# AER-RC/monoRTM

Measured on AMD Instinct MI355X. Metric: (wavenumber x layer x line) optical-depth evals/sec, higher is better.
Workload: dtype f64; 1 GPU; c4: configs[3] whole: 1024 synthetic sonde profiles x 64 layers x 50 channels x 500 lines, f64, profile-sharded over 1 GPU(s): 1024 profiles on this rank; layers=64, wavenumbers=50, lines=500, nmol=7, launch=3 stream launches, parallelism=profile-sharded x1

## Files before the change

### monortm_amd/csrc/api.hip

```cpp
#include <algorithm>
#include <atomic>
#include <chrono>
#include <cmath>
#include <cstdlib>
#include <cstdio>
#include <cstring>
#include <dlfcn.h>
#include <functional>
#include <string>
#include <vector>

#include "device_common.hpp"
#include "line_table.hpp"
#include "modm_plan.hpp"
#include "lineshape.hpp"
#include "tables/monortm_tables.h"

namespace {
using namespace monortm_dev;

thread_local std::string g_init_error;

struct Ctx {
    int device = 0;
    int cus = 256;
    size_t phys_cap = 2ull << 30, far_cap = 1ull << 30;
    std::vector<Ctx *> shards;
    struct Opt : ModmPlanOpt {
        int ms_ablate = 0;
        double jac_dt = MONORTM_JAC_DT, jac_dlnw = MONORTM_JAC_DLNW;
    } opt;
    void *comm = nullptr;
    int comm_rank = 0, comm_world = 1;
    bool has_lines = false;
    int real_kind = 8;
    std::string err;
    monortm::LineTable host;
    DevLines lines{};
    DevTables tables{};
    std::vector<void *> owned;
    int *errflag = nullptr;
    void *partial = nullptr;
    monortm_dev::MwCache mw_cache;
    void *phys = nullptr;
    size_t phys_bytes = 0;
    void *far = nullptr;
    size_t far_bytes = 0;
    double lines_per_cm = 0.;
    bool no_physics_pass = false;
    hipStream_t far_stream = nullptr;
    hipEvent_t far_ev[2] = {nullptr, nullptr};
    double lc_frac = 0.;
    const int *ms_slot_base = nullptr;
    int ms_slot_host[MXMOL + 1] = {0};
    void *ms_scratch = nullptr;
    unsigned short *ms_reach = nullptr;
    size_t ms_scratch_bytes = 0;
    double *osum = nullptr;
    size_t osum_elems = 0;
    DevXsec xs{};
    std::vector<void *> xs_buf;
    struct Stage {
        void *p = nullptr;
        size_t bytes = 0;
    };
    Stage stage[12];
    void *jac_ws = nullptr;
    size_t jac_ws_bytes = 0;
    struct Obs {
        int handle = 0;
        int npath = 0, nwn = 0, nview = 0, nchan = 0;
        void *dev = nullptr;
        const int *view_start = nullptr, *mstart = nullptr, *mlane = nullptr;
        const double *wpath = nullptr, *mw = nullptr;
        std::vector<int> shard;
    };
    static constexpr int kMaxObs = 16;
    Obs obs[kMaxObs];
    hipStream_t hs = nullptr;
    int *errflag_host = nullptr;
    struct {
        const void *dev = nullptr, *host = nullptr;
// ... 25 lines not shown
    do {                                                                                             \
        hipError_t e_ = (call);                                                                      \
        if (e_ != hipSuccess) {                                                                      \
            (c)->err = std::string(#call) + ": " + hipGetErrorString(e_);                            \
            return MONORTM_EHIP;                                                                     \
        }                                                                                            \
    } while (0)

constexpr size_t kKernelCopyMax = 4u << 20;
__global__ __launch_bounds__(256) void copy16_kernel(const uint4 *__restrict__ src, uint4 *__restrict__ dst, size_t n16,
                                                     const uint4 *__restrict__ src2, uint4 *__restrict__ dst2, size_t n16b,
                                                     const int *flag_src, int *flag_dst) {
    for (size_t i = (size_t)blockIdx.x * 256 + threadIdx.x; i < n16; i += (size_t)gridDim.x * 256) dst[i] = src[i];
    if (blockIdx.x == gridDim.x - 1)
        for (size_t i = threadIdx.x; i < n16b; i += 256) dst2[i] = src2[i];
    if (flag_dst && blockIdx.x == 0 && threadIdx.x == 0) *flag_dst = *flag_src;
}
hipError_t move_arena(void *dst, const void *src, size_t bytes, hipMemcpyKind kind, hipStream_t s, const int *flag_src = nullptr,
                      int *flag_dst = nullptr, void *dst2 = nullptr, const void *src2 = nullptr, size_t bytes2 = 0) {
    if (bytes <= kKernelCopyMax) {
        const size_t n16 = bytes / 16;
        const unsigned blocks = (unsigned)std::min<size_t>(256, std::max<size_t>(1, (n16 + 255) / 256));
        hipLaunchKernelGGL(copy16_kernel, dim3(blocks), dim3(256), 0, s, static_cast<const uint4 *>(src), static_cast<uint4 *>(dst), n16,
                           static_cast<const uint4 *>(src2), static_cast<uint4 *>(dst2), bytes2 / 16, flag_src, flag_dst);
        return hipGetLastError();
    }
    hipError_t e = hipMemcpyAsync(dst, src, bytes, kind, s);
    if (e == hipSuccess && flag_dst) e = hipMemcpyAsync(flag_dst, flag_src, sizeof(int), hipMemcpyDeviceToHost, s);
    if (e == hipSuccess && bytes2) e = hipMemcpyAsync(dst2, src2, bytes2, hipMemcpyDefault, s);
    return e;
}

void comm_release(Ctx *c);

int set_option(Ctx *c, const char *name, const char *value) {
    const std::string n = name ? name : "", v = value ? value : "";
    const bool autov = v.empty() || v == "auto";
    long iv = 0;
    double dv = 0.;
    bool isint = false, isdbl = false;
    if (!autov) {
        char *end = nullptr;
        iv = strtol(v.c_str(), &end, 10);
        isint = end && end != v.c_str() && *end == '\0';
        end = nullptr;
        dv = strtod(v.c_str(), &end);
        isdbl = end && end != v.c_str() && *end == '\0';
    }
    if (n == "nslice" && (autov || (isint && iv >= 1 && iv <= 16))) c->opt.nslice = autov ? 0 : (int)iv;
    else if (n == "fair" && (autov || (isint && (iv == 0 || iv == 1)))) c->opt.fair = autov ? -1 : (int)iv;
    else if (n == "tile_waves" && (autov || (isint && (iv == 1 || iv == 2 || iv == 4)))) c->opt.tile_waves = autov ? 0 : (int)iv;
    else if (n == "far_levels" && (autov || (isint && iv >= 0 && iv <= FAR_MAXLEV))) c->opt.far_levels = autov ? -1 : (int)iv;
    else if (n == "lines_kernel" && (autov || v == "wn" || v == "ms")) c->opt.lines_ms = autov ? -1 : (v == "ms" ? 1 : 0);
#ifdef MONORTM_EXPERIMENT
    else if (n == "ms_ablate" && isint && iv >= 0 && iv <= 9) c->opt.ms_ablate = (int)iv;
#endif
    else if (n == "finish" && (autov || v == "generic")) c->opt.finish_generic = autov ? 0 : 1;
    else if (n == "ms_items" && (autov || (isint && (iv == 64 || iv == 128 || iv == 192 || iv == 256)))) c->opt.ms_items = autov ? 0 : (int)iv;
    else if ((n == "jac_dt" || n == "jac_dlnw") && (autov || (isdbl && std::isfinite(dv) && dv > 0. && (n == "jac_dt" || dv < 1.)))) {
        if (n == "jac_dt") c->opt.jac_dt = autov ? MONORTM_JAC_DT : dv;
        else c->opt.jac_dlnw = autov ? MONORTM_JAC_DLNW : dv;
    }
    else { c->err = "unknown option or value: " + n + " = " + v; return MONORTM_EARG; }
    return MONORTM_OK;
}

template <class T>
int upload(Ctx *c, const T *src, size_t n, const T **dst) {
    void *p = nullptr;
    const size_t bytes = std::max<size_t>(n, 1) * sizeof(T);
    HIPCHK(c, hipMalloc(&p, bytes));
    c->owned.push_back(p);
    if (n) HIPCHK(c, hipMemcpy(p, src, n * sizeof(T), hipMemcpyHostToDevice));
    *dst = static_cast<const T *>(p);
    return MONORTM_OK;
}

void prof_begin(Ctx *c, hipStream_t s, int k, Ctx::Ev &ev) {
    ev.k = -1;
    if (!((c->profiling >> k) & 1)) return;
    if (c->prof_stride > 1 && (c->prof_calls[k]++ % c->prof_stride) != 0) return;
    auto take = [&](hipEvent_t *e) {
        if (!c->event_pool.empty()) { *e = c->event_pool.back(); c->event_pool.pop_back(); }
        else hipEventCreate(e);
    };
    take(&ev.a);
    take(&ev.b);
    ev.k = k;
    hipEventRecord(ev.a, s);
}
void prof_end(Ctx *c, hipStream_t s, Ctx::Ev &ev) {
    if (ev.k < 0) return;
    hipEventRecord(ev.b, s);
    c->events.push_back(ev);
}

hipError_t grow(void **p, size_t *have, size_t need, size_t elem = 1) {
    if (need <= *have) return hipSuccess;
    hipError_t e = *p ? hipFree(*p) : hipSuccess;
    *p = nullptr;
    *have = 0;
    if (e == hipSuccess) e = hipMalloc(p, need * elem);
    if (e == hipSuccess) *have = need;
    else *p = nullptr;
    return e;
}
// ... 615 lines not shown
    {
        int iso_max[MXMOL + 1] = {0};
        for (size_t i = 0; i < h.meta.size(); i++) {
            const int mol = (int)(h.meta[i] & 63u), iso = (int)((h.meta[i] >> 6) & 15u);
            if (mol >= 1 && mol <= MXMOL) iso_max[mol] = std::max(iso_max[mol], std::max(iso, 1));
        }
        int acc = 0;
        for (int m = 0; m < MXMOL; m++) { c->ms_slot_host[m] = acc; acc += std::min(iso_max[m + 1], 9); }
        c->ms_slot_host[MXMOL] = acc;
        if ((rc = upload(c, c->ms_slot_host, (size_t)MXMOL + 1, &c->ms_slot_base))) return failed(rc);
    }
    DevTables &t = c->tables;
#define UT(field, arr) if ((rc = upload(c, arr, sizeof(arr) / sizeof(arr[0]), &t.field))) return failed(rc)
    UT(self296, MT_SELF296); UT(self260, MT_SELF260); UT(frgn296, MT_FRGN296); UT(fco2, MT_FCO2);
    UT(n2c296, MT_N2RT296_C); UT(n2sf296, MT_N2RT296_SF); UT(n2c220, MT_N2RT220_C); UT(n2sf220, MT_N2RT220_SF);
    UT(xfac_rhu, MT_XFAC_RHU); UT(xfacco2, MT_XFACCO2); UT(tdep_bandhead, MT_TDEP_BANDHEAD);
    UT(tips_qoft, TIPS_QOFT); UT(smass, ISO_SMASS); UT(tips_isonm, TIPS_ISONM); UT(tips_offset, TIPS_OFFSET);
    UT(o3ch_x, MT_O3CH_X); UT(o3ch_y, MT_O3CH_Y); UT(o3ch_z, MT_O3CH_Z); UT(o3hh0, MT_O3HH0); UT(o3hh1, MT_O3HH1);
    UT(o3hh2, MT_O3HH2); UT(o3huv, MT_O3HUV); UT(o2f_x, MT_O2F_XO2); UT(o2f_t, MT_O2F_XO2T); UT(o2inf1, MT_O2INF1);
    UT(o2inf3, MT_O2INF3); UT(o2vis, MT_O2VIS); UT(o2fuv, MT_O2FUV); UT(n2f_272, MT_N2F_272); UT(n2f_228, MT_N2F_228);
    UT(n2f_ah2o, MT_N2F_AH2O); UT(n2f1, MT_N2F1);
#undef UT
    {
        std::vector<double> q296(sizeof(TIPS_QOFT) / sizeof(double) / 119);
        for (size_t i = 0; i < q296.size(); i++) q296[i] = tips_atob(296., &TIPS_QOFT[i * 119]);
        if ((rc = upload(c, q296.data(), q296.size(), &t.tips_q296))) return failed(rc);
    }
    {
        const struct { const double *t296, *tlow; const double **out; int n; } lr[3] = {
            {t.self296, t.self260, &t.lr_self, MT_SELF296_NPT},
            {t.n2c296, t.n2c220, &t.lr_n2c, MT_N2RT296_NPT},
            {t.n2sf296, t.n2sf220, &t.lr_n2sf, MT_N2RT296_NPT}};
        for (const auto &e : lr) {
            void *p = nullptr;
            if (hipMalloc(&p, sizeof(double) * (size_t)e.n) != hipSuccess) { c->err = "hipMalloc(log-ratio table) failed"; return failed(MONORTM_EHIP); }
            c->owned.push_back(p);
            launch_logratio(e.t296, e.tlow, static_cast<double *>(p), e.n, nullptr);
            *e.out = static_cast<const double *>(p);
        }
        if (hipGetLastError() != hipSuccess || hipDeviceSynchronize() != hipSuccess) { c->err = "log-ratio tables could not be formed"; return failed(MONORTM_EHIP); }
    }
    void *ef = nullptr;
    if (hipMalloc(&ef, sizeof(int)) != hipSuccess || hipMemset(ef, 0, sizeof(int)) != hipSuccess) { c->err = "hipMalloc(errflag) failed"; return failed(MONORTM_EHIP); }
    c->owned.push_back(ef);
    c->errflag = static_cast<int *>(ef);
    if (hipDeviceSynchronize() != hipSuccess) { c->err = "device set-up failed"; return failed(MONORTM_EHIP); }
    if (hipStreamCreateWithFlags(&c->hs, hipStreamNonBlocking) != hipSuccess ||
        hipHostMalloc(reinterpret_cast<void **>(&c->errflag_host), sizeof(int), hipHostMallocDefault) != hipSuccess) {
        c->err = "stream / pinned flag of the host-buffer entry points could not be created";
        return failed(MONORTM_EHIP);
    }
    if (const char *e = getenv("MONORTM_HOST_TIMING")) c->host_timing = e[0] == '1';
    if (getenv("MONORTM_FINISH_GENERIC")) c->opt.finish_generic = 1;
    for (const char *k : {"lines_kernel", "nslice", "fair", "tile_waves", "far_levels", "ms_items",
#ifdef MONORTM_EXPERIMENT
                          "ms_ablate",
#endif
                         }) {
        std::string env = "MONORTM_" + std::string(k);
        for (char &ch : env) ch = (char)toupper((unsigned char)ch);
        if (const char *e = getenv(env.c_str()))
            if (set_option(c, k, e)) { c->err = env + ": " + c->err; return failed(MONORTM_EARG); }
    }
    if (c->host_timing && !g_timing_ctx) {
        g_timing_ctx = c;
        static bool registered = false;
        if (!registered) { atexit([] { if (g_timing_ctx) print_host_timing(g_timing_ctx); }); registered = true; }
    }
    *out = c;
    return MONORTM_OK;
}

void monortm_hip_finalize(void *ctx) {
    Ctx *c = static_cast<Ctx *>(ctx);
    if (!c) return;
    if (!c->shards.empty()) {
        for (Ctx *sh : c->shards) monortm_hip_finalize(sh);
        delete c;
        return;
    }
    print_host_timing(c);
    if (g_timing_ctx == c) g_timing_ctx = nullptr;
    DeviceGuard guard;
    hipSetDevice(c->device);
    for (auto &e : c->events) { hipEventDestroy(e.a); hipEventDestroy(e.b); }
    for (auto &e : c->event_pool) hipEventDestroy(e);
    comm_release(c);
    if (c->hs) hipStreamDestroy(c->hs);
    if (c->errflag_host) hipHostFree(c->errflag_host);
    for (void *p : c->owned) hipFree(p);
    if (c->partial) hipFree(c->partial);
    if (c->osum) hipFree(c->osum);
    if (c->ms_scratch) hipFree(c->ms_scratch);
    for (void *p : c->xs_buf) hipFree(p);
    if (c->phys) hipFree(c->phys);
    if (c->far) hipFree(c->far);
    if (c->far_stream) hipStreamDestroy(c->far_stream);
    for (hipEvent_t e : c->far_ev)
        if (e) hipEventDestroy(e);
    c->mw_cache.release();
    if (c->jac_ws) hipFree(c->jac_ws);
    for (auto &ob : c->obs)
        if (ob.dev) hipFree(ob.dev);
    for (int i = 0; i < 12; i++)
        if (c->stage[i].p) {
            if (i % 2 == 0) hipHostFree(c->stage[i].p);
            else hipFree(c->stage[i].p);
// ... 348 lines not shown
    int rc = check_modm_args(c, nprof, nwn, nlay_max, nmol, ibrd, ixsect, vends[1]);
    if (rc) return rc;
    ModmArgs a{};
    a.real_kind = c->real_kind;
    a.nprof = nprof; a.nwn = nwn; a.nlay_max = nlay_max; a.nmol = nmol; a.ibrd = ibrd;
    a.dvset = dvset; a.sclcpl = sclcpl; a.sclhw = sclhw; a.y0res = y0res;
    for (int i = 0; i < 7; i++) a.cntnm[i] = cntnm_fac[i];
    a.wn = wn; a.P = P; a.T = T; a.CLW = CLW; a.WKL = WKL; a.WBRODL = WBRODL; a.nlay = nlay;
    a.O = O; a.O_BY_MOL = O_BY_MOL; a.OC = OC; a.O_CLW = O_CLW; a.errflag = c->errflag;
    if (ixsect == 1) {
        if (!XAMNT || !ODXSEC) { c->err = "IXSECT = 1: XAMNT / ODXSEC missing"; return MONORTM_EARG; }
        if (c->xs.nxs < 1) { c->err = "IXSECT = 1: no cross-section tables on this context (monortm_hip_xsec_tables)"; return MONORTM_EARG; }
        a.XAMNT = XAMNT; a.ODXSEC = ODXSEC; a.nxs = c->xs.nxs;
    }

    ModmPlanIn in{};
    in.nprof = nprof; in.nwn = nwn; in.nlay_max = nlay_max; in.nmol = nmol; in.real_kind = c->real_kind; in.ibrd = ibrd; in.ixsect = ixsect;
    in.v1 = vends[0]; in.v2 = vends[1];
    in.nlines = (long long)c->host.size(); in.lines_per_cm = c->lines_per_cm; in.lc_frac = c->lc_frac; in.any_brd = c->host.any_brd;
    in.ms_nslot = c->ms_slot_host[nmol];
    in.cus = c->cus; in.phys_cap = c->phys_cap; in.far_cap = c->far_cap;
    in.opt = c->opt;
    in.no_physics_pass = c->no_physics_pass;
    ModmPlan pl;
    const char *why = nullptr;
    if ((rc = modm_plan(in, &pl, &why))) { c->err = why; return rc; }

    HIPCHK(c, grow(&c->partial, &c->partial_elems, pl.partial_elems, (size_t)c->real_kind));
    a.nslice = pl.nslice;
    a.partial = c->partial;
    a.fair = pl.fair;
    if (pl.need_osum) {
        HIPCHK(c, grow(reinterpret_cast<void **>(&c->osum), &c->osum_elems, pl.osum_elems, sizeof(double)));
        a.osum = c->osum;
    }
    Ctx::Ev ev{};
    prof_begin(c, s, 0, ev);
    if ((rc = dense_passes(c, pl, a, s))) return rc;
    MsArgs ms = pl.ms;
    if (pl.use_ms) {
        HIPCHK(c, grow(&c->ms_scratch, &c->ms_scratch_bytes, lines_ms_scratch(ms, (long long)ms.npg * nlay_max)));
        const size_t nl4 = (std::max<size_t>(c->host.size(), 1) + 3) / 4 * 4;
        if (!c->ms_reach) {
            void *p = nullptr;
            HIPCHK(c, hipMalloc(&p, 6 * nl4));
            c->owned.push_back(p);
            c->ms_reach = static_cast<unsigned short *>(p);
        }
        ms.reach = c->ms_reach;
        ms.near0 = reinterpret_cast<float *>(c->ms_reach + nl4);
        ms.scratch = c->ms_scratch;
        ms.slot_base = c->ms_slot_base;
        ms.ablate = c->opt.ms_ablate;
    }
    const dim3 grid(pl.grid[0], pl.grid[1], pl.grid[2]);
    if (pl.use_ms && pl.ms_nprof < nprof) {
        ModmArgs am = a, aw = a;
        am.nprof = pl.ms_nprof;
        const size_t st = (size_t)pl.ms_nprof * nlay_max;
        auto shift = [](const void *p, size_t elems) { return p ? static_cast<const void *>(static_cast<const double *>(p) + elems) : nullptr; };
        aw.nprof = nprof - pl.ms_nprof;
        aw.P = shift(a.P, st); aw.T = shift(a.T, st); aw.CLW = shift(a.CLW, st); aw.WBRODL = shift(a.WBRODL, st);
        aw.WKL = shift(a.WKL, st * nmol);
        aw.nlay = a.nlay + pl.ms_nprof;
        aw.O = const_cast<void *>(shift(a.O, st * nwn)); aw.O_CLW = const_cast<void *>(shift(a.O_CLW, st * nwn));
        aw.O_BY_MOL = const_cast<void *>(shift(a.O_BY_MOL, st * nmol * nwn));
        aw.OC = const_cast<void *>(shift(a.OC, st * MONORTM_NCONT * nwn));
        aw.osum = a.osum ? a.osum + st * nwn : nullptr;
        launch_lines_ms(am, c->lines, c->tables, ms, pl.use_brd, s);
        launch_lines(aw, c->lines, c->tables, pl.nw, pl.wpl, pl.use_brd, dim3(grid.x, (unsigned)aw.nprof, grid.z), pl.dyn_lds, s);
    } else if (pl.use_ms) launch_lines_ms(a, c->lines, c->tables, ms, pl.use_brd, s);
    else launch_lines(a, c->lines, c->tables, pl.nw, pl.wpl, pl.use_brd, grid, pl.dyn_lds, s);
    prof_end(c, s, ev);
    HIPCHK(c, hipGetLastError());
    prof_begin(c, s, 1, ev);
    if (ixsect == 1) launch_xsec(a, c->xs, s);
    a.slices_reduced = pl.slices_reduced;
    if (pl.slices_reduced) launch_reduce_slices(a, s);
    if (pl.mw) {
        const hipError_t e = launch_finish_mw(a, c->tables, vends[0], vends[1], pl.V1ABS, pl.V2ABS, pl.NPTABS, c->mw_cache, s);
        if (e != hipSuccess) {
            c->err = std::string("launch_finish_mw: ") + (c->mw_cache.why ? c->mw_cache.why : hipGetErrorString(e));
            return c->mw_cache.why ? MONORTM_EUNSUPPORTED : MONORTM_EHIP;
        }
    } else HIPCHK(c, launch_finish(a, c->tables, pl.V1ABS, pl.V2ABS, pl.NPTABS, pl.csize, pl.high, pl.par, pl.fin_threads, pl.fin_lds, pl.lds_sets, s));
    c->finish_launches[pl.finish_variant]++;
    prof_end(c, s, ev);
    HIPCHK(c, hipGetLastError());
    return MONORTM_OK;
}

int monortm_hip_rtm_dev(void *ctx, int nprof, int nwn, const double *wn, const int *nlay, int nlay_max, const int *irt,
                        int iout, const void *T, const void *TZ, const void *O, void *tmpsfc, const void *emiss,
                        const void *reflc, void *RUP, void *RDN, void *TRTOT, void *RAD, void *TB, void *TMR,
                        void *stream) {
    Ctx *c = static_cast<Ctx *>(ctx);
    if (!c) return null_ctx();
    if (!c->shards.empty()) return multi_only_host(c);
    hipStream_t s = (hipStream_t)stream;
    if (!wn || !nlay || !irt || !T || !TZ || !O || !tmpsfc || !emiss || !reflc || !RUP || !RDN || !TRTOT || !RAD || !TB) { c->err = "null array argument"; return MONORTM_EARG; }
    if (int rcd = check_device(c)) return rcd;
    if (nprof < 1 || nwn < 1 || nlay_max < 1) { c->err = "bad nprof/nwn/nlay_max"; return MONORTM_EARG; }
    RtmArgs a{};
    a.real_kind = c->real_kind;
    a.nprof = nprof; a.nwn = nwn; a.nlay_max = nlay_max; a.iout = iout;
    a.wn = wn; a.T = T; a.TZ = TZ; a.O = O; a.emiss = emiss; a.reflc = reflc; a.nlay = nlay; a.irt = irt;
// ... 850 lines not shown
```

### monortm_amd/csrc/device_common.hpp

```cpp
#pragma once
#include <hip/hip_runtime.h>

#if (defined(FAR_ABL_HOT) || defined(FAR_ABL_STEPS) || defined(FAR_ABL_TRANS) || defined(MONORTM_ABLATE_LOOP) || defined(MONORTM_ABLATE_EVAL) || \
     defined(MONORTM_ABLATE_VOIGT) || defined(MONORTM_ABLATE_ZSEARCH) || defined(MONORTM_ABLATE_EXP4) || defined(MONORTM_ABLATE_COUPLE) ||     \
     defined(MONORTM_NO_CLAMP_GUARD) || defined(MONORTM_NO_UNIFIED) || defined(MONORTM_NO_VSCAN) ||              \
     defined(MONORTM_NO_HALF) || defined(MONORTM_NO_FULL) || defined(MONORTM_NO_CHUNKFAR) || defined(MONORTM_NO_SGL_TSKIP) || defined(LINES_TIMING) || \
     defined(LINES_CLASS_STATS) || defined(MW_TIMING)) &&                                                                                          \
    !defined(MONORTM_EXPERIMENT)
#error "a timing-experiment / A-B switch of monortm_amd is defined: such builds are measurements, not the product - add -DMONORTM_EXPERIMENT=1"
#endif

#include <cstdint>

#include "../../include/monortm_hip.h"

namespace monortm_dev {

#define K_PI 3.1415926535898
#define K_PLANCK 6.62606876E-27
#define K_BOLTZ 1.3806503E-16
#define K_CLIGHT 2.99792458E+10
#define K_AVOGAD 6.02214199E+23
#define K_RADCN1 1.191042722E-12
#define K_RADCN2 1.4387752
// ... 224 lines not shown
    const double TRd = exp_cw(-ODTd);
    const double bnum = fma(pade, bbz, bb);
    RDN = fma((TRd * emis) * bnum, rp1, RDN);
    sumexp = fma((bnum * rp1) * TRd, emis, sumexp);
    if (up) {
        const double TRu = exp_cw(-ODTu);
        RUP = fma((TRu * emis) * fma(pade, bb_top, bb), rp1, RUP);
        ODTu = ODTu + ODVI;
    }
}
__device__ __forceinline__ void rtm_combine(int irt, double VV, double RUP, double RDN, double sumexp, double ODTOT, double ESFC, double RSFC,
                                            double SURFRAD, double COSMOS, bool want_tb, bool want_tmr, double &TRTOT, double &RAD,
                                            double &TB, double &TMR) {
#pragma clang fp contract(off)
    const double c3 = K_RADCN1 * (VV * VV * VV);
    TRTOT = exp(-ODTOT);
    TMR = 0.;
    if (want_tmr) {
        const double radtmr = sumexp / (1. - exp(-1 * ODTOT));
        TMR = K_RADCN2 * VV / log(c3 / radtmr + 1.);
    }
    const double sky = fma(TRTOT, COSMOS, RDN);
    RAD = 0.;
    if (irt == 1) RAD = fma(TRTOT, fma(RSFC, sky, ESFC * SURFRAD), RUP);
    if (irt == 2) RAD = fma(TRTOT, sky, RUP);
    if (irt == 3) RAD = sky;
    TB = want_tb ? K_RADCN2 * VV / log(c3 / RAD + 1.) : 0.;
}
__device__ __forceinline__ double doppler_factor(double M, double T) {
    return sqrt(2. * log(2.) * ((K_BOLTZ * T) / (M / K_AVOGAD))) / K_CLIGHT;
}

template <typename R>
__host__ __device__ inline const R *rp(const void *p) { return static_cast<const R *>(p); }
template <typename R>
__host__ __device__ inline R *wp(void *p) { return static_cast<R *>(p); }

#define MS_WPS 5
#define MS_MAXSTEPS 4
constexpr int MS_HOTA_BYTES = 32;
struct MsArgs {
    int G, LPS, CL, nsteps;
    int spp;
    int sa_stride;
    int npg;
    int nslot;
    int inv_cl;
    int inv_lps;
    const int *slot_base;
    void *scratch;
    unsigned short *reach;
    float *near0;
    int ablate;
};
size_t lines_ms_scratch(const MsArgs &ms, long long nwg);
void launch_lines_ms(const ModmArgs &a, const DevLines &L, const DevTables &tb, const MsArgs &ms, bool ibrd, hipStream_t s);

void launch_physics(const ModmArgs &a, const DevLines &L, const DevTables &tb, int nlines, bool ibrd, hipStream_t s);
void launch_far_plan(const ModmArgs &a, const DevLines &L, const DevTables &tb, hipStream_t s);
void launch_far(const ModmArgs &a, const DevLines &L, const DevTables &tb, double rho_tile, double lines_per_cm, long long *launches,
                hipStream_t s);
void launch_lines(const ModmArgs &a, const DevLines &L, const DevTables &tb, int nw, int wpl, bool ibrd, dim3 grid, size_t dyn_lds,
                  hipStream_t s);
hipError_t launch_finish(const ModmArgs &a, const DevTables &tb, double V1ABS, double V2ABS, int NPTABS, int csize, bool high,
                         bool par, int threads, size_t lds, int lds_sets, hipStream_t s);
void launch_reduce_slices(const ModmArgs &a, hipStream_t s);
void launch_logratio(const double *t296, const double *tlow, double *out, int n, hipStream_t s);
struct MwCache {
    struct Entry {
        double key[5];
        void *items;
        hipEvent_t built;
        hipStream_t stream;
        bool ready;
        unsigned long long last_use;
    };
    static constexpr int kMax = 8;
    Entry e[kMax];
    int n = 0;
    unsigned long long clock = 0;
    const char *why = nullptr;
    void release();
};
hipError_t launch_finish_mw(const ModmArgs &a, const DevTables &tb, double V1, double V2, double V1ABS, double V2ABS, int NPTABS, MwCache &cache,
                            hipStream_t s);
void launch_kat(int which, int n, const double *in, const double *tab, double *out, int *errflag, const DevTables &tb, hipStream_t s);
void launch_xsec(const ModmArgs &a, const DevXsec &x, hipStream_t s);
void launch_rtm(const RtmArgs &a, hipStream_t s);
void launch_rtm_scan(const RtmScanArgs &a, hipStream_t s);
void launch_jac_perturb(const JacPerturbArgs &a, hipStream_t s);
void launch_rtm_jac(const RtmJacArgs &a, bool full, hipStream_t s);
void launch_rtm_scan_jac(const RtmScanJacArgs &a, bool full, hipStream_t s);
void launch_rtm_obs_jac(const RtmObsJacArgs &a, bool full, int out_kind, hipStream_t s);
void launch_rtm_obs(const RtmObsArgs &a, int out_kind, hipStream_t s);

}
```

### monortm_amd/csrc/lines_device.hpp

```cpp
#pragma once
#include "lineshape.hpp"
#include "lines_asm.hpp"

namespace {
using namespace monortm_dev;

__device__ __forceinline__ unsigned long long uni64(unsigned long long x) {
    const unsigned lo = __builtin_amdgcn_readfirstlane((unsigned)x), hi = __builtin_amdgcn_readfirstlane((unsigned)(x >> 32));
    return ((unsigned long long)hi << 32) | lo;
}

__device__ __forceinline__ double frcp(double x) {
    const double r = __builtin_amdgcn_rcp(x);
    return fma(fma(-x, r, 1.0), r, r);
}
__device__ __forceinline__ float frcp(float x) { return __builtin_amdgcn_rcpf(x); }
__device__ __forceinline__ double frcp_any(double x) {
    double r = __builtin_amdgcn_rcp(x);
    r = fma(fma(-x, r, 1.0), r, r);
    return fma(fma(-x, r, 1.0), r, r);
}

template <int CTRL, int ROW_MASK>
__device__ __forceinline__ double dpp_move(double v, double idle = 0.) {
// ... 54 lines not shown
        p = fma(p, r, 1.0);
        p = fma(p, r, 1.0);
        return ldexp(p, (int)n);
    }
#endif
    double p = 1.0 / 6227020800.0;
    p = fma(p, r, 1.0 / 479001600.0);
    p = fma(p, r, 1.0 / 39916800.0);
    p = fma(p, r, 1.0 / 3628800.0);
    p = fma(p, r, 1.0 / 362880.0);
    p = fma(p, r, 1.0 / 40320.0);
    p = fma(p, r, 1.0 / 5040.0);
    p = fma(p, r, 1.0 / 720.0);
    p = fma(p, r, 1.0 / 120.0);
    p = fma(p, r, 1.0 / 24.0);
    p = fma(p, r, 1.0 / 6.0);
    p = fma(p, r, 0.5);
    p = fma(p, r, 1.0);
    p = fma(p, r, 1.0);
    return ldexp(p, (int)n);
}

#ifdef MONORTM_EXP_SGPR_CONSTANTS
__device__ __forceinline__ void horner4_s(double (&p)[4], const double (&r)[4], double c) {
    asm("v_fma_f64 %0, %0, %4, %8\n\tv_fma_f64 %1, %1, %5, %8\n\tv_fma_f64 %2, %2, %6, %8\n\tv_fma_f64 %3, %3, %7, %8"
        : "+v"(p[0]), "+v"(p[1]), "+v"(p[2]), "+v"(p[3])
        : "v"(r[0]), "v"(r[1]), "v"(r[2]), "v"(r[3]), "s"(c));
}
__device__ __forceinline__ void exp_prep4(const double (&x)[4], double (&out)[4]) {
    double n[4], r[4], p[4];
#pragma unroll
    for (int i = 0; i < 4; i++) {
        n[i] = rint(x[i] * 1.44269504088896338700e+00);
        r[i] = fma(-n[i], 6.93147180369123816490e-01, x[i]);
        r[i] = fma(-n[i], 1.90821492927058770002e-10, r[i]);
        p[i] = 1.0 / 6227020800.0;
    }
    horner4_s(p, r, 1.0 / 479001600.0);
    horner4_s(p, r, 1.0 / 39916800.0);
    horner4_s(p, r, 1.0 / 3628800.0);
    horner4_s(p, r, 1.0 / 362880.0);
    horner4_s(p, r, 1.0 / 40320.0);
    horner4_s(p, r, 1.0 / 5040.0);
    horner4_s(p, r, 1.0 / 720.0);
    horner4_s(p, r, 1.0 / 120.0);
    horner4_s(p, r, 1.0 / 24.0);
    horner4_s(p, r, 1.0 / 6.0);
#pragma unroll
    for (int i = 0; i < 4; i++) {
        p[i] = fma(p[i], r[i], 0.5);
        p[i] = fma(p[i], r[i], 1.0);
        p[i] = fma(p[i], r[i], 1.0);
        out[i] = ldexp(p[i], (int)n[i]);
    }
}
#endif

__device__ __forceinline__ double tanh_pos(double x) {
    if (x < 0.125) {
        const double z = x * x;
        double p = 21844.0 / 6081075.0;
        p = fma(p, z, -1382.0 / 155925.0);
        p = fma(p, z, 62.0 / 2835.0);
        p = fma(p, z, -17.0 / 315.0);
        p = fma(p, z, 2.0 / 15.0);
        p = fma(p, z, -1.0 / 3.0);
        return fma(x * z, p, x);
    }
    const double e = exp_prep(-2.0 * x);
    return (1.0 - e) / (1.0 + e);
}


__device__ __forceinline__ double fma_clamp0(double a, double b, double c) {
    double r;
    asm("v_fma_f64 %0, %1, %2, -%3 clamp" : "=v"(r) : "v"(a), "v"(b), "v"(c));
    return r;
}

template <int KIND, bool M2, bool TEST>
__device__ __forceinline__ double eval_one_fast(const HotA h, const double pb_or_lim, double WN) {
    const double d = WN - h.xnu;
    const double den1 = fma(d, d, h.hw2);
    const double cutlim = (KIND == 1) ? h.pa : 25.;
    const bool live = !(fabs(d) > cutlim);
    double term;
    if constexpr (KIND == 0 && !M2 && TEST) return fma_clamp0(h.a2, frcp(den1), h.pa);
    if constexpr (KIND == 0 && M2) {
        const double dp = WN + h.xnu;
        const double den2 = fma(dp, dp, h.hw2);
        const double q = h.a2 * frcp(den1 * den2);
        return fma_clamp0(q, den2, h.pa) + fma_clamp0(q, den1, pb_or_lim);
    }
    if (KIND == 2) {
        const double f = fma(-(d * d), 1.0 / 625., 2.);
        term = fma(-h.pa, f, h.a2 * frcp(den1));
    } else if (!M2) {
        term = (KIND == 0) ? fma(h.a2, frcp(den1), -h.pa) : h.a2 * frcp(den1);
    } else {
        const double dp = WN + h.xnu;
        const double m2f = (dp <= ((KIND == 1) ? pb_or_lim : 25.)) ? 1.0 : 0.0;
        const double den2 = fma(dp, dp, h.hw2);
        const double num = fma(m2f, den1, den2);
        const double t = h.a2 * num;
        if (KIND == 0) term = fma(t, frcp(den1 * den2), -fma(m2f, pb_or_lim, h.pa));
        else term = t * frcp(den1 * den2);
// ... 1184 lines not shown
```

### monortm_amd/csrc/lines_ms_kernel.hip

```cpp
#define MONORTM_EXP_SGPR_CONSTANTS 1
#include "lines_device.hpp"
#include "lines_ms_asm.hpp"
#include "modm_plan.hpp"
#include "ms_reach.hpp"

namespace {
using namespace monortm_dev;

constexpr int WPS = MS_WPS;
static_assert(MS_REACH_SLOTS == MS_WPS, "ms_reach.hpp forms one bit per wavenumber of a lane");

__device__ __forceinline__ void ms_sync() {
    __builtin_amdgcn_fence(__ATOMIC_RELEASE, "wavefront");
    __builtin_amdgcn_wave_barrier();
    __builtin_amdgcn_fence(__ATOMIC_ACQUIRE, "wavefront");
}
__device__ __forceinline__ void ms_sync_global() {
    __builtin_amdgcn_fence(__ATOMIC_RELEASE, "workgroup");
    __builtin_amdgcn_s_waitcnt(0);
    __builtin_amdgcn_wave_barrier();
    __builtin_amdgcn_fence(__ATOMIC_ACQUIRE, "workgroup");
}

struct MsState {
    const HotA *sA;
    const HotB *gB;
    const ColdLine *gC;
    int item0;
};
struct MsSpec { unsigned long long w[MS_MAXSTEPS]; };
__device__ __forceinline__ bool ms_own(const MsSpec &sp, int item) {
    unsigned long long x = sp.w[0];
#pragma unroll
    for (int t = 1; t < MS_MAXSTEPS; t++) x = ((item >> 6) == t) ? sp.w[t] : x;
    return (x >> (item & 63)) & 1ull;
}
__device__ __forceinline__ HotB ms_hotb(const MsState &st, const MsSpec &sp, int j, const HotA &h) {
    if (ms_own(sp, st.item0 + j)) return st.gB[j];
    return HotB{h.pa, -1., 0., 1.};
}

template <int KIND>
__device__ __forceinline__ void ms_voigt_flush(const HotA *sA, const HotB *gB, const ColdLine *gC, const MsArgs &ms, const unsigned short *vq, int n,
                                               const double (&W)[WPS], int mol, double (&S)[WPS], int *errflag) {
    const int lane = (int)__lane_id();
    const unsigned rec = (lane < n) ? vq[lane] : 0u;
    const int j = (int)((rec >> 9) & 63u), kk = (int)((rec >> 6) & 7u), owner = (int)(rec & 63u);
    double WNi = __shfl(W[0], owner);
#pragma unroll
    for (int k = 1; k < WPS; k++) {
        const double wk = __shfl(W[k], owner);
        WNi = (kk == k) ? wk : WNi;
    }
    double val = 0.;
    if (lane < n) {
        const int so = owner / ms.LPS;
        const HotA h = sA[so * ms.sa_stride + j];
        const HotB b = gB[so * ms.CL + j];
        const ColdLine c = gC[so * ms.CL + j];
        const double SLS = lsf_sdvoigt(mol, (int)((c.info >> 6) & 3), 1.0, 1.0, b.c1 * c.hw, b.gp1 - 1., c.hw, WNi, h.xnu, c.hwd,
                                       (double)c.sdep, cold_xl3(c, mol, errflag), errflag);
        double lor;
// ... 217 lines not shown
                for (int m = 0; m < nmol; m++) obm[(size_t)m * nwn + ce + LPS * k] = 0.;
    }
    if (lay == 0) {
        if (prof_ok && ce == 0 && (nl_e < 1 || nl_e > a.nlay_max)) atomicOr(a.errflag, ERRBIT_ARG);
        if (pg == 0)
            for (int i = lane; i + 1 < nwn; i += 64) {
                const double w0 = a.wn[i], w1 = a.wn[i + 1];
                if (w1 < w0) atomicOr(a.errflag, ERRBIT_ARG);
                if (a.dvset != 0. && !(fabs(w1 - (a.wn[0] + (double)(i + 1) * a.dvset)) <= 0.25 * fabs(a.dvset))) atomicOr(a.errflag, ERRBIT_ARG);
            }
    }
    if (__builtin_amdgcn_ballot_w64(act_e) == 0ull) return -1;
    const unsigned pass_e = (unsigned)(se / ms.spp), sub_e = (unsigned)se - pass_e * (unsigned)ms.spp;
    l.sRole[lane] = (int)((unsigned)se | ((unsigned)ce << 8) | (kvalid << 16) | ((unsigned)prof_ok << 24) | ((unsigned)act_e << 25) | (pass_e << 26) | (sub_e << 28));

    l.sWn[lane] = a.wn[min(lane, nwn - 1)];
    if (lane <= nmol) l.sSlot[lane] = ms.slot_base[lane];
    {
        const double Pk = act_e ? static_cast<const double *>(a.P)[pl_e] : K_P0, Tk = act_e ? static_cast<const double *>(a.T)[pl_e] : K_T0,
                     wbrod = act_e ? static_cast<const double *>(a.WBRODL)[pl_e] : 1.;
        const double *wk = static_cast<const double *>(a.WKL) + pl_e * nmol;
        const double RADCT = K_PLANCK * K_CLIGHT / K_BOLTZ;
        const double XN0 = (K_P0 / (K_BOLTZ * K_T0)) * 1.E+3;
        const double Xn = (Pk / (K_BOLTZ * Tk)) * 1.E+3;
        double WTOT = 0.;
        for (int m = 0; m < nmol; m++) WTOT += act_e ? wk[m] : 0.;
        WTOT = WTOT + wbrod;
        const double RP = Pk / K_P0, RP2 = RP * RP;
        const double RT = Tk / K_T0, RHORAT = Xn / XN0;
        const int ILC = (Tk < 250.0) ? 1 : ((Tk < 296.0) ? 2 : 3);
        const double tlo = (ILC == 1) ? 200.0 : (ILC == 2 ? 250.0 : 296.0);
        const double RECTLC = (ILC == 1) ? 1.0 / (250.0 - 200.0) : ((ILC == 2) ? 1.0 / (296.0 - 250.0) : 1.0 / (340.0 - 296.0));
        const double TMPDIF = Tk - tlo;
        const double lnRT = log(RT);
        const double cTk = RADCT / Tk, cT0 = RADCT / K_T0, dTinv = 1.0 / K_T0 - 1.0 / Tk;
        if (lane_in) {
            double *ly = l.sLay + se * 20;
            if (ce == 0) {
                ly[0] = RHORAT; ly[1] = RP; ly[2] = RP2; ly[3] = lnRT; ly[4] = cTk; ly[5] = cT0; ly[6] = dTinv;
                ly[7] = RECTLC; ly[8] = TMPDIF; ly[9] = WTOT; ly[17] = (double)ILC; ly[18] = Tk; ly[19] = act_e ? 1. : 0.;
            }
            for (int j = ce; j < MXBRD; j += LPS) ly[10 + j] = RHORAT * ((act_e && j < nmol) ? wk[j] : 0.) / WTOT;
            for (int m = ce; m < nmol; m += LPS) l.sW[se * nmol + m] = act_e ? wk[m] : 0.;
        }
        {
            double *gR = reinterpret_cast<double *>(static_cast<char *>(ms.scratch) + (size_t)blockIdx.x * ms_scratch_per_wg(G, CL) +
                                                    (size_t)G * CL * (sizeof(HotB) + sizeof(ColdLine)));
#pragma unroll 1
            for (int k = 0; k < WPS; k++) {
                const double w = a.wn[min(ce + LPS * k, nwn - 1)];
                gR[k * 64 + lane] = w * tanh_pos((RADCT * w) / (2 * Tk));
            }
        }
        if (act_e && ce == 0 && (Tk < 70. || Tk > 3000.)) atomicOr(a.errflag, ERRBIT_TEMP);
    }
    if (lane < nmol) { l.sLo[lane] = 0x7fffffff; l.sOff[lane + 1] = 0; }
    for (int i = lane; i < 2 * G; i += 64) l.sA[(i >> 1) * ms.sa_stride + CL + (i & 1)] = HotA{0., 1., 0., 0.};
    ms_sync();

    if (lane == 0) {
        unsigned long long dense = 0ull;
        for (int s = 0; s < G; s++) {
            const double rh = l.sLay[s * 20];
            if (l.sLay[s * 20 + 19] != 0. && !(rh <= MS_REACH_RHO)) dense = 1ull;
        }
        l.sMask[4 + MS_MAXSTEPS + WPS] = dense;
    }
    for (int i = lane; i < G * nmol; i += 64) {
        const int s = i / nmol, m = i - s * nmol, mol = m + 1;
        const double *ly = l.sLay + s * 20;
        if (ly[19] == 0.) continue;
        const double wkq = l.sW[s * nmol + m];
        int lo = L.mol_start[m + 1], hi = L.mol_start[m + 2];
        if (wkq == 0.) continue;
        const double RHORAT = ly[0], WTOT = ly[9], Tk = ly[18];
        if ((mol != 7 || !((L.lc_mask >> 7) & 1ull)) && ((L.sorted_mask >> mol) & 1ull) && WTOT == WTOT && RHORAT == RHORAT && Tk == Tk) {
            const double pad = L.max_abs_shift * fmax(RHORAT, 1.0) + 1e-6;
            const double vlo = l.sWn[0] - 25.0 - pad, vhi = l.sWn[63] + 25.0 + pad;
            int l0 = lo, l1 = hi;
            while (l0 < l1) { const int mid = (l0 + l1) >> 1; if (L.vnu[mid] < vlo) l0 = mid + 1; else l1 = mid; }
            const int first = l0;
            l1 = hi;
            while (l0 < l1) { const int mid = (l0 + l1) >> 1; if (L.vnu[mid] <= vhi) l0 = mid + 1; else l1 = mid; }
            lo = first;
            hi = l0;
        }
        if (hi > lo) {
            atomicMin(&l.sLo[m], lo);
            atomicMax(&l.sOff[m + 1], hi);
        }
    }
    ms_sync();
    if (lane == 0) {
        int acc = 0;
        l.sOff[0] = 0;
        for (int m = 0; m < nmol; m++) {
            const int cnt = (l.sOff[m + 1] > l.sLo[m]) ? l.sOff[m + 1] - l.sLo[m] : 0;
            acc += cnt;
            l.sOff[m + 1] = acc;
        }
    }
    ms_sync();
    for (int i = lane; i < G * nslot; i += 64) {
        const int s = i / nslot, slot = i - s * nslot;
        int m = 0;
        while (m + 1 < nmol && l.sSlot[m + 1] <= slot) m++;
        const int mol = m + 1, iso = slot - l.sSlot[m] + 1;
        const double *ly = l.sLay + s * 20;
        double sc = 0., dop = 0.;
        if (ly[19] != 0. && l.sOff[m + 1] > l.sOff[m]) {
            const double Tk = ly[18];
            if (!(Tk < 70. || Tk > 3000.)) {
                bool bad = false;
                sc = tips_scor(tb.tips_isonm, tb.tips_offset, tb.tips_qoft, tb.tips_q296, mol, iso, Tk, &bad);
                if (bad) atomicOr(a.errflag, ERRBIT_TEMP);
            }
            const double M = tb.smass[(mol - 1) * 9 + iso - 1];
            if (M > 0.) dop = doppler_factor(M, Tk);
        }
        l.sScor[i] = sc;
        l.sDop[i] = dop;
    }
    if (act_e)
        for (int m = 0; m < nmol; m++)
            if (l.sOff[m + 1] == l.sOff[m]) {
#pragma unroll
                for (int k = 0; k < WPS; k++)
                    if ((kvalid >> k) & 1u) obm[(size_t)m * nwn + ce + LPS * k] = 0.;
            }
    ms_sync();
    return l.sOff[nmol];
}

template <bool IBRD>
__device__ __forceinline__ void ms_prepare(const unsigned long long *sKseg, int base, int mchunk, int total, HotB *gB, ColdLine *gC) {
    extern __shared__ __attribute__((aligned(16))) double dyn_lds[];
    const kseg_t ks = ms_kseg_from(*sKseg);
    const ModmArgs &a = *(const ModmArgs *)ks;
    const DevLines &L = *(const DevLines *)(ks + KA_LINES);
    const MsArgs &ms = *(const MsArgs *)(ks + KA_MS);
    const int G = ms.G, CL = ms.CL, nmol = a.nmol, nslot = ms.nslot;
    const MsLds ld = ms_lds(dyn_lds, G, ms.sa_stride, nmol, nslot, nullptr);
    const int lane = threadIdx.x;
    const int sub = (int)(((unsigned)lane * (unsigned)ms.inv_cl) >> 16), l = lane - sub * CL;
    const bool lane_in = sub < ms.spp;
    const bool lin = lane_in && base + l < total;
    int m = mchunk, idx = 0, slot0 = 0;
    LineFields lf{0., 0., 0.f, 0.f, 0.f, 0.f, 0.f, 0u};
    float near0 = 0.f;
    if (lin) {
        const int v = base + l;
        while (ld.sOff[m + 1] <= v) m++;
        idx = ld.sLo[m] + (v - ld.sOff[m]);
        slot0 = ld.sSlot[m];
        if constexpr (IBRD) lf.meta = L.meta[idx];
        else lf = load_line_fields(L, idx);
        near0 = ms.near0[idx];
    }
    const uint32_t meta = lf.meta;
    const bool plain = ((meta >> 10) & 3u) == 0u && ((meta >> 13) & 3u) == 0u;
    const bool all_plain = __builtin_amdgcn_ballot_w64(lin && !plain) == 0ull;
#pragma unroll 1
    for (int t = 0; t < ms.nsteps; t++) {
        const int s = t * ms.spp + sub;
        const bool s_in = lane_in && s < G;
        const bool in = lin && s_in && ld.sLay[s * 20 + 19] != 0.;
        const int item = s * CL + l;
        HotA hA{0., 1., 0., 0.};
        unsigned flag = 0u;
        bool special = false;
        if (in) {
            int idxp = idx, mp = m;
            uint32_t metap = meta;
            if constexpr (IBRD) asm volatile("" : "+v"(idxp), "+v"(mp), "+v"(metap));
            const int molp = mp + 1, isop = (metap >> 6) & 15;
            const double *ly = ld.sLay + s * 20;
            LayerScalars lys;
            lys.ILC = (int)ly[17];
            lys.RHORAT = ly[0]; lys.RP = ly[1]; lys.RP2 = ly[2]; lys.lnRT = ly[3]; lys.cTk = ly[4]; lys.cT0 = ly[5];
            lys.dTinv = ly[6]; lys.RECTLC = ly[7]; lys.TMPDIF = ly[8];
            double rho7[MXBRD];
#pragma unroll
            for (int j = 0; j < MXBRD; j++) rho7[j] = IBRD ? ly[10 + j] : 0.;
            const double rho_self = (molp <= MXBRD) ? ly[10 + molp - 1] : lys.RHORAT * ld.sW[s * nmol + molp - 1] / ly[9];
            const int sl = s * nslot + slot0;
            const double XIPSF = isop ? ld.sScor[sl + isop - 1] : 0.;
            const double dopfac = isop ? ld.sDop[sl + isop - 1] : ld.sDop[sl];
            LineFields lfp = lf;
            if constexpr (IBRD) lfp = load_line_fields(L, idxp);
            lfp.meta = metap;
            HotB hB;
            ColdLine cC;
            bool fAL, fM2, fV, fY;
            if (all_plain) {
                const LinePhys ph = line_physics_core<IBRD, true>(phys_params(a, L), idxp, molp, lfp, lys, rho_self, rho7, XIPSF, dopfac);
                const double near_lb = (double)near0 * (1. - 1e-6) - fabs(ph.xnu - lfp.xnu0) - 1e-9;
                line_records<double, true>(a, L, idxp, mp, metap, ph, ld.sW + s * nmol, ld.sWn, 64, hA, hB, cC, fAL, fM2, fV, fY, near_lb);
            } else {
                const LinePhys ph = line_physics_core<IBRD>(phys_params(a, L), idxp, molp, lfp, lys, rho_self, rho7, XIPSF, dopfac);
                const double near_lb = (double)near0 * (1. - 1e-6) - fabs(ph.xnu - lfp.xnu0) - 1e-9;
                line_records<double>(a, L, idxp, mp, metap, ph, ld.sW + s * nmol, ld.sWn, 64, hA, hB, cC, fAL, fM2, fV, fY, near_lb);
            }
            flag = (fAL ? 0u : 1u) | (fM2 ? 2u : 0u) | (fV ? 4u : 0u) | (fY ? 8u : 0u);
            special = fV || fY;
            if (special) {
                gB[item] = hB;
                gC[item] = cC;
            }
        }
        if (s_in) {
            ld.sA[s * ms.sa_stride + l] = hA;
            ld.sFlag[item] = (unsigned char)flag;
        }
        const unsigned long long bs = __builtin_amdgcn_ballot_w64(special);
        if (lane == 0) ld.sMask[4 + t] = bs;
    }
// ... 179 lines not shown
```

Baseline: 1596 billion evals/s.

## Add fused multi-step line preparation with batched exponentials in ms kernel

Adds a fast path in ms_prepare that, when every line in the wave is plain, not broadened and within the first MXBRD molecules, prepares all 2 or 3 layer steps at once. The exponentials for those steps are computed together through a hand-written batched Horner polynomial that uses scalar-register coefficients, and the path writes HotA entries and flags directly. If any lane hits an unusual case the wave falls back to the existing per-step loop. It also adds an option to force the old passes and rewrites the temperature check to catch NaN, at the cost of more register pressure and duplicated logic.

```diff
diff --git a/monortm_amd/csrc/api.hip b/monortm_amd/csrc/api.hip
--- a/monortm_amd/csrc/api.hip
+++ b/monortm_amd/csrc/api.hip
@@ -28,6 +28,7 @@
     std::vector<Ctx *> shards;
     struct Opt : ModmPlanOpt {
         int ms_ablate = 0;
+        int ms_prepare = MS_PREPARE_FUSED;
         double jac_dt = MONORTM_JAC_DT, jac_dlnw = MONORTM_JAC_DLNW;
     } opt;
     void *comm = nullptr;
@@ -159,6 +160,7 @@
     else if (n == "tile_waves" && (autov || (isint && (iv == 1 || iv == 2 || iv == 4)))) c->opt.tile_waves = autov ? 0 : (int)iv;
     else if (n == "far_levels" && (autov || (isint && iv >= 0 && iv <= FAR_MAXLEV))) c->opt.far_levels = autov ? -1 : (int)iv;
     else if (n == "lines_kernel" && (autov || v == "wn" || v == "ms")) c->opt.lines_ms = autov ? -1 : (v == "ms" ? 1 : 0);
+    else if (n == "ms_prepare" && (autov || v == "fused" || v == "passes")) c->opt.ms_prepare = v == "passes" ? MS_PREPARE_PASSES : MS_PREPARE_FUSED;
 #ifdef MONORTM_EXPERIMENT
     else if (n == "ms_ablate" && isint && iv >= 0 && iv <= 9) c->opt.ms_ablate = (int)iv;
 #endif
@@ -880,7 +882,7 @@
     }
     if (const char *e = getenv("MONORTM_HOST_TIMING")) c->host_timing = e[0] == '1';
     if (getenv("MONORTM_FINISH_GENERIC")) c->opt.finish_generic = 1;
-    for (const char *k : {"lines_kernel", "nslice", "fair", "tile_waves", "far_levels", "ms_items",
+    for (const char *k : {"lines_kernel", "nslice", "fair", "tile_waves", "far_levels", "ms_items", "ms_prepare",
 #ifdef MONORTM_EXPERIMENT
                           "ms_ablate",
 #endif
@@ -1335,6 +1337,7 @@
         ms.scratch = c->ms_scratch;
         ms.slot_base = c->ms_slot_base;
         ms.ablate = c->opt.ms_ablate;
+        ms.prepare = c->opt.ms_prepare;
     }
     const dim3 grid(pl.grid[0], pl.grid[1], pl.grid[2]);
     if (pl.use_ms && pl.ms_nprof < nprof) {
diff --git a/monortm_amd/csrc/device_common.hpp b/monortm_amd/csrc/device_common.hpp
--- a/monortm_amd/csrc/device_common.hpp
+++ b/monortm_amd/csrc/device_common.hpp
@@ -300,7 +300,10 @@
     unsigned short *reach;
     float *near0;
     int ablate;
-};
+    int prepare;
+};
+#define MS_PREPARE_FUSED 0
+#define MS_PREPARE_PASSES 1
 size_t lines_ms_scratch(const MsArgs &ms, long long nwg);
 void launch_lines_ms(const ModmArgs &a, const DevLines &L, const DevTables &tb, const MsArgs &ms, bool ibrd, hipStream_t s);
 
diff --git a/monortm_amd/csrc/lines_device.hpp b/monortm_amd/csrc/lines_device.hpp
--- a/monortm_amd/csrc/lines_device.hpp
+++ b/monortm_amd/csrc/lines_device.hpp
@@ -130,6 +130,51 @@
         p[i] = fma(p[i], r[i], 1.0);
         p[i] = fma(p[i], r[i], 1.0);
         out[i] = ldexp(p[i], (int)n[i]);
+    }
+}
+__device__ __forceinline__ void horner_n_s(double (&p)[8], const double (&r)[8], double c) {
+    asm("v_fma_f64 %0, %0, %8, %16\n\tv_fma_f64 %1, %1, %9, %16\n\tv_fma_f64 %2, %2, %10, %16\n\tv_fma_f64 %3, %3, %11, %16\n\t"
+        "v_fma_f64 %4, %4, %12, %16\n\tv_fma_f64 %5, %5, %13, %16\n\tv_fma_f64 %6, %6, %14, %16\n\tv_fma_f64 %7, %7, %15, %16"
+        : "+v"(p[0]), "+v"(p[1]), "+v"(p[2]), "+v"(p[3]), "+v"(p[4]), "+v"(p[5]), "+v"(p[6]), "+v"(p[7])
+        : "v"(r[0]), "v"(r[1]), "v"(r[2]), "v"(r[3]), "v"(r[4]), "v"(r[5]), "v"(r[6]), "v"(r[7]), "s"(c));
+}
+__device__ __forceinline__ void horner_n_s(double (&p)[12], const double (&r)[12], double c) {
+    asm("v_fma_f64 %0, %0, %12, %24\n\tv_fma_f64 %1, %1, %13, %24\n\tv_fma_f64 %2, %2, %14, %24\n\tv_fma_f64 %3, %3, %15, %24\n\t"
+        "v_fma_f64 %4, %4, %16, %24\n\tv_fma_f64 %5, %5, %17, %24\n\tv_fma_f64 %6, %6, %18, %24\n\tv_fma_f64 %7, %7, %19, %24\n\t"
+        "v_fma_f64 %8, %8, %20, %24\n\tv_fma_f64 %9, %9, %21, %24\n\tv_fma_f64 %10, %10, %22, %24\n\tv_fma_f64 %11, %11, %23, %24"
+        : "+v"(p[0]), "+v"(p[1]), "+v"(p[2]), "+v"(p[3]), "+v"(p[4]), "+v"(p[5]), "+v"(p[6]), "+v"(p[7]), "+v"(p[8]), "+v"(p[9]),
+          "+v"(p[10]), "+v"(p[11])
+        : "v"(r[0]), "v"(r[1]), "v"(r[2]), "v"(r[3]), "v"(r[4]), "v"(r[5]), "v"(r[6]), "v"(r[7]), "v"(r[8]), "v"(r[9]), "v"(r[10]),
+          "v"(r[11]), "s"(c));
+}
+template <int N>
+__device__ __forceinline__ void exp_prep_n(const double (&x)[N], double (&out)[N]) {
+    double r[N], p[N];
+    int n[N];
+#pragma unroll
+    for (int i = 0; i < N; i++) {
+        const double nd = rint(x[i] * 1.44269504088896338700e+00);
+        r[i] = fma(-nd, 6.93147180369123816490e-01, x[i]);
+        r[i] = fma(-nd, 1.90821492927058770002e-10, r[i]);
+        p[i] = 1.0 / 6227020800.0;
+        n[i] = (int)nd;
+    }
+    horner_n_s(p, r, 1.0 / 479001600.0);
+    horner_n_s(p, r, 1.0 / 39916800.0);
+    horner_n_s(p, r, 1.0 / 3628800.0);
+    horner_n_s(p, r, 1.0 / 362880.0);
+    horner_n_s(p, r, 1.0 / 40320.0);
+    horner_n_s(p, r, 1.0 / 5040.0);
+    horner_n_s(p, r, 1.0 / 720.0);
+    horner_n_s(p, r, 1.0 / 120.0);
+    horner_n_s(p, r, 1.0 / 24.0);
+    horner_n_s(p, r, 1.0 / 6.0);
+#pragma unroll
+    for (int i = 0; i < N; i++) {
+        p[i] = fma(p[i], r[i], 0.5);
+        p[i] = fma(p[i], r[i], 1.0);
+        p[i] = fma(p[i], r[i], 1.0);
+        out[i] = ldexp(p[i], n[i]);
     }
 }
 #endif
diff --git a/monortm_amd/csrc/lines_ms_kernel.hip b/monortm_amd/csrc/lines_ms_kernel.hip
--- a/monortm_amd/csrc/lines_ms_kernel.hip
+++ b/monortm_amd/csrc/lines_ms_kernel.hip
@@ -8,6 +8,11 @@
 using namespace monortm_dev;
 
 constexpr int WPS = MS_WPS;
+#if defined(MONORTM_ABLATE_EXP4) || defined(MONORTM_ABLATE_ZSEARCH) || defined(MONORTM_ABLATE_VOIGT) || defined(MONORTM_NO_CLAMP_GUARD)
+constexpr bool MS_HAS_TRIP = false;
+#else
+constexpr bool MS_HAS_TRIP = true;
+#endif
 static_assert(MS_REACH_SLOTS == MS_WPS, "ms_reach.hpp forms one bit per wavenumber of a lane");
 
 __device__ __forceinline__ void ms_sync() {
@@ -331,7 +336,7 @@
                 gR[k * 64 + lane] = w * tanh_pos((RADCT * w) / (2 * Tk));
             }
         }
-        if (act_e && ce == 0 && (Tk < 70. || Tk > 3000.)) atomicOr(a.errflag, ERRBIT_TEMP);
+        if (act_e && ce == 0 && !(Tk >= 70. && Tk <= 3000.)) atomicOr(a.errflag, ERRBIT_TEMP);
     }
     if (lane < nmol) { l.sLo[lane] = 0x7fffffff; l.sOff[lane + 1] = 0; }
     for (int i = lane; i < 2 * G; i += 64) l.sA[(i >> 1) * ms.sa_stride + CL + (i & 1)] = HotA{0., 1., 0., 0.};
@@ -409,6 +414,77 @@
             }
     ms_sync();
     return l.sOff[nmol];
+}
+
+template <int NS>
+__device__ __forceinline__ bool ms_prepare_trip(const MsArgs &ms, const MsLds &ld, int nslot, bool lin, int m, int slot0, const LineFields &lf,
+                                                float near0) {
+#pragma clang fp contract(off)
+    const int G = ms.G, CL = ms.CL, spp = ms.spp;
+    int lane = (int)__lane_id();
+    asm volatile("" : "+v"(lane));
+    const int sub = (int)(((unsigned)lane * (unsigned)ms.inv_cl) >> 16), l = lane - sub * CL;
+    const bool lane_in = sub < spp;
+    const int mol = m + 1, iso = (lf.meta >> 6) & 15;
+    const double RADCT = K_PLANCK * K_CLIGHT / K_BOLTZ;
+    const double xnu0 = lf.xnu0, s0adj = lf.s0adj, alpf = lf.alfa, delt = lf.pshift, E = lf.epp, XTILD = lf.tmpalf;
+    const double RE = RADCT * E;
+    double alps = lf.hwhm;
+    if (mol == 1 && alps == 0.) alps = 5 * alpf;
+    const double near_s = (double)near0 * (1. - 1e-6);
+    const int oself = 10 + min(mol, MXBRD) - 1, oslot = slot0 + (iso ? iso - 1 : 0);
+    const double w0 = ld.sWn[0], w63 = ld.sWn[63];
+    double Xnu[NS], xa[4 * NS], ex[4 * NS];
+#pragma unroll
+    for (int t = 0; t < NS; t++) {
+        const int s = t * spp + sub;
+        const double *ly = ld.sLay + ((lane_in & (s < G)) ? s : 0) * 20;
+        const double RHORAT = ly[0], lnRT = ly[3], cTk = ly[4], cT0 = ly[5], dTinv = ly[6];
+        Xnu[t] = xnu0 + (delt * RHORAT);
+        xa[4 * t] = RE * dTinv;
+        xa[4 * t + 1] = -(Xnu[t] * cTk);
+        xa[4 * t + 2] = -(Xnu[t] * cT0);
+        xa[4 * t + 3] = XTILD * lnRT;
+    }
+    exp_prep_n<4 * NS>(xa, ex);
+    bool bad = false;
+#pragma unroll
+    for (int t = 0; t < NS; t++) {
+        const int s = t * spp + sub;
+        const bool s_in = lane_in & (s < G);
+        const int sc = s_in ? s : 0;
+        const double *ly = ld.sLay + sc * 20;
+        const bool in = lin & s_in & (ly[19] != 0.);
+        const double RHORAT = ly[0], rho_self = ly[oself];
+        const double scor = ld.sScor[sc * nslot + oslot], dopfac = ld.sDop[sc * nslot + oslot];
+        const double XIPSF = iso ? scor : 0.;
+        const double S = s0adj * ex[4 * t] * XIPSF;
+        const double STILD = S * ((1 + ex[4 * t + 1]) * frcp_any(Xnu[t] * (1 - ex[4 * t + 2])));
+        const double rtx = ex[4 * t + 3];
+        const double alfa0i = alpf * rtx, hwhmsi = alps * rtx;
+        const double HW = alfa0i * (RHORAT - rho_self) + hwhmsi * rho_self;
+        const double HWD = Xnu[t] * dopfac;
+        const double c1 = 0., g = 0., wsc = 1.0;
+        const double zsum = HW + HWD, zthr = 0.99 * zsum;
+        const bool z_gt = HW > zthr * (1. + 1e-12), z_lt = HW < zthr * (1. - 1e-12);
+        const double A2 = STILD * HW * (1.0 / K_PI);
+        const double HW2 = HW * HW;
+        const double p = A2 * frcp_any(625. + HW2);
+        const double A2w = A2 * wsc;
+        const double pa = (mol == 7) ? 25. : ((mol == 2) ? p : p * ((1. + c1 * 25.) + g)) * wsc;
+        const double near_lb = near_s - fabs(Xnu[t] - xnu0) - 1e-9;
+        const bool fY = (mol != 7) & (mol != 2) & !((A2w >= 0.) & (HW2 == HW2) & (A2 <= 0.25 * HW2));
+        bad |= in & ((!z_gt & !(z_lt & (near_lb > 100. * HWD))) | fY);
+        const bool fM2 = (mol != 2) & (w0 + Xnu[t] <= 25.);
+        const bool fAL = !(fabs(w0 - Xnu[t]) > 25.) & !(fabs(w63 - Xnu[t]) > 25.);
+        if (s_in) {
+            ld.sA[s * ms.sa_stride + l] = in ? HotA{Xnu[t], HW2, A2w, pa} : HotA{0., 1., 0., 0.};
+            ld.sFlag[s * CL + l] = in ? (unsigned char)((fAL ? 0u : 1u) | (fM2 ? 2u : 0u)) : (unsigned char)0;
+        }
+    }
+    if (__builtin_amdgcn_ballot_w64(bad) != 0ull) return false;
+    if ((sub == 0) & (l < NS)) ld.sMask[4 + l] = 0ull;
+    return true;
 }
 
 template <bool IBRD>
@@ -439,8 +515,15 @@
     const uint32_t meta = lf.meta;
     const bool plain = ((meta >> 10) & 3u) == 0u && ((meta >> 13) & 3u) == 0u;
     const bool all_plain = __builtin_amdgcn_ballot_w64(lin && !plain) == 0ull;
+    bool done = false;
+    if constexpr (MS_HAS_TRIP && !IBRD) {
+        if (all_plain && ms.prepare != MS_PREPARE_PASSES && __builtin_amdgcn_ballot_w64(lin && m >= MXBRD) == 0ull) {
+            if (ms.nsteps == 3) done = ms_prepare_trip<3>(ms, ld, nslot, lin, m, slot0, lf, near0);
+            else if (ms.nsteps == 2) done = ms_prepare_trip<2>(ms, ld, nslot, lin, m, slot0, lf, near0);
+        }
+    }
 #pragma unroll 1
-    for (int t = 0; t < ms.nsteps; t++) {
+    for (int t = done ? ms.nsteps : 0; t < ms.nsteps; t++) {
         const int s = t * ms.spp + sub;
         const bool s_in = lane_in && s < G;
         const bool in = lin && s_in && ld.sLay[s * 20 + 19] != 0.;
```

New measurement: 1633 billion evals/s (median of 6 runs). 1.02x the previous value.
